# LuoGroup2023/PanTax

Hardware: AMD Instinct MI355X
Metric: PAO wall-time (s) + Mreads/s: packed reads + DB (graphs and their unique-trio index) resident in HBM -> abundance tables; the metric's own GAF -> abundance quantity is value_gaf_to_tables (files -> tables, never `value`) (higher is better)
Workload: dtype int64+f64

## Files before the change

include/pantax_hip.h:

```cpp
#ifndef PANTAX_HIP_H
#define PANTAX_HIP_H
#include <stddef.h>
#include <stdint.h>
#ifdef __cplusplus
extern "C" {
#endif

typedef enum {
    PANTAX_HIP_OK = 0,
    PANTAX_HIP_E_INVALID = -1,
    PANTAX_HIP_E_HIP = -2,
    PANTAX_HIP_E_NO_DEVICE = -3,
    PANTAX_HIP_E_LIMIT = -4,
    PANTAX_HIP_E_SOLVER = -5,
    PANTAX_HIP_E_IO = -6,
    PANTAX_HIP_E_STATE = -7
} pantax_hip_status;

typedef struct pantax_hip_ctx pantax_hip_ctx;
typedef struct pantax_hip_db pantax_hip_db;
typedef struct pantax_hip_reads pantax_hip_reads;

int pantax_hip_init(pantax_hip_ctx **out, const int *device_ids, int n_devices);
void pantax_hip_destroy(pantax_hip_ctx *ctx);
// ... 216 lines not shown
int pantax_hip_reads_load_gaf(pantax_hip_ctx *ctx, const char *path, pantax_hip_reads **reads_out, pantax_hip_gaf **gaf_out);
int pantax_hip_reads_set_flags(pantax_hip_ctx *ctx, pantax_hip_reads *reads, const uint8_t *flags);
void pantax_hip_gaf_free(pantax_hip_gaf *gaf);

typedef struct pantax_hip_graph pantax_hip_graph;
int pantax_hip_graph_load(const char *path, int format, pantax_hip_graph **out, const char **err_out);
int pantax_hip_graph_view(const pantax_hip_graph *g, uint64_t *n_nodes, uint64_t *n_haps, const int64_t **node_len,
                          const uint64_t **path_off, const uint32_t **path_nodes, const char *const **hap_names);
void pantax_hip_graph_free(pantax_hip_graph *g);

int pantax_hip_format_f64(double v, char *buf, size_t cap);

int pantax_hip_strain_node_stats(pantax_hip_ctx *ctx, pantax_hip_db *db, double *amax_out, uint32_t *nvalid_out, double *nzsum_out,
                                 uint32_t *nzcnt_out);

int pantax_hip_timing_enable(pantax_hip_ctx *ctx, int on);
int pantax_hip_timing_reset(pantax_hip_ctx *ctx);
int pantax_hip_timing_filter(pantax_hip_ctx *ctx, const char *name);
int pantax_hip_timing_get(pantax_hip_ctx *ctx, int cap, const char **names_out, uint64_t *launches_out,
                          double *total_ms_out);
int pantax_hip_sync(pantax_hip_ctx *ctx);

#ifdef __cplusplus
}
#endif
#endif
```

pantax_amd/_ffi.py:

```python
import ctypes as C
import os

import numpy as np

_HERE = os.path.dirname(os.path.abspath(__file__))
LIB_PATH = os.path.join(_HERE, "lib", "libpantax_hip.so")
_lib = None

SYMBOLS = [
    "pantax_hip_init", "pantax_hip_destroy", "pantax_hip_last_error", "pantax_hip_version", "pantax_hip_set_option",
    "pantax_hip_db_upload", "pantax_hip_db_upload_parts", "pantax_hip_db_free", "pantax_hip_reads_upload", "pantax_hip_reads_free",
    "pantax_hip_bin_reads", "pantax_hip_species_profile", "pantax_hip_db_reset", "pantax_hip_abundance_filter",
    "pantax_hip_trio_index", "pantax_hip_trio_get", "pantax_hip_node_coverage",
    "pantax_hip_strain_profile", "pantax_hip_strain_node_stats", "pantax_hip_pao_solve", "pantax_hip_pao_solve_batch", "pantax_hip_profile", "pantax_hip_profile_step", "pantax_hip_profile_step_enqueue", "pantax_hip_profile_step_collect", "pantax_hip_trio_index_prefetch", "pantax_hip_sort_rows",
    "pantax_hip_sample_ranks", "pantax_hip_chacha_block", "pantax_hip_gaf_filter", "pantax_hip_db_save_images", "pantax_hip_db_load_images",
    "pantax_hip_gaf_load", "pantax_hip_gaf_load_device", "pantax_hip_reads_load_gaf", "pantax_hip_reads_set_flags", "pantax_hip_gaf_view", "pantax_hip_gaf_free",
    "pantax_hip_graph_load", "pantax_hip_graph_view", "pantax_hip_graph_free", "pantax_hip_format_f64",
    "pantax_hip_read_strains", "pantax_hip_reads_route_pack", "pantax_hip_route_buffer", "pantax_hip_route_free", "pantax_hip_reads_from_routed",
    "pantax_hip_timing_enable", "pantax_hip_timing_filter", "pantax_hip_timing_reset", "pantax_hip_timing_get", "pantax_hip_sync",
]


class PantaxHipError(RuntimeError):
    def __init__(self, code, msg):
        super().__init__("pantax_hip error %d: %s" % (code, msg))
        self.code = code


class Graphs(C.Structure):
# ... 102 lines not shown
```

pantax_amd/csrc/api_core.cpp:

```cpp
#include <algorithm>
#include <chrono>
#include <cstdio>
#include <cstdlib>
#include <cstring>
#include <memory>
#include <numeric>
#include <string>
#include "common.hpp"

using namespace ptx;

extern "C" {

int pantax_hip_db_upload(pantax_hip_ctx *ctx, const pantax_hip_graphs *g, pantax_hip_db **out) {
    if (!ctx || !g || !out) return PANTAX_HIP_E_INVALID;
    *out = nullptr;
    PTX_ENTER(ctx);
    uint32_t S = g->n_species;
    if (S == 0) return fail(ctx, PANTAX_HIP_E_INVALID, "db_upload: n_species == 0");
    std::unique_ptr<pantax_hip_db> db(new pantax_hip_db());
    db->S = S;
    if (!g->node_len) {
        std::vector<uint32_t> order(S), rs(S), re(S);
        std::iota(order.begin(), order.end(), 0u);
// ... 290 lines not shown
    lap("node-block runs");
    PTX_TRY(node_haps_build(ctx, db));
    lap("node -> haplotypes");
    PTX_HIP(ctx, db->d_trio_first.alloc(1));
    PTX_HIP(ctx, db->d_trio_ent.alloc(2));
    PTX_HIP(ctx, db->d_trio_bases.alloc(1));
    PTX_HIP(ctx, db->d_active.alloc(S));
    PTX_HIP(ctx, hipStreamSynchronize(ctx->stream));
    return 0;
}

}

extern "C" {

void pantax_hip_db_free(pantax_hip_ctx *ctx, pantax_hip_db *db) {
    std::unique_lock<std::recursive_mutex> lk;
    if (ctx) lk = std::unique_lock<std::recursive_mutex>(ctx->mu);
    bool idle = false;
    if (ctx) {
        (void)hipSetDevice(ctx->device);
        idle = hipStreamSynchronize(ctx->stream) == hipSuccess;
        if (ctx->stream2) idle = hipStreamSynchronize(ctx->stream2) == hipSuccess && idle;
    }
    if (idle) { DevCacheIdleFrees scope; delete db; }
    else delete db;
}

int pantax_hip_reads_upload(pantax_hip_ctx *ctx, const pantax_hip_packed_reads *r, pantax_hip_reads **out) {
    if (!ctx || !r || !out) return PANTAX_HIP_E_INVALID;
// ... 92 lines not shown
```

pantax_amd/csrc/api_strain.cpp:

```cpp
#include <algorithm>
#include <chrono>
#include <cstdio>
#include <cstdlib>
#include <cmath>
#include <cstring>
#include <memory>
#include "lad.hpp"
#include "primitives.hpp"

using namespace ptx;

namespace {

inline double round2(double x) { return std::round(x * 100.0) / 100.0; }

struct StrainRaw {
    const uint32_t *nnz, *nvalid, *nzcnt, *sp_pat_off, *counts;
    const double *meanf, *amax, *nzsum, *x1, *x2, *obj1, *obj2;
    const int32_t *hap_bit, *sp_p, *st1, *st2, *it1, *it2;
    const uint8_t *fixed2, *need2;
    const unsigned long long *ratio;
};

struct ArenaLayout {
// ... 271 lines not shown

int pantax_hip_strain_node_stats(pantax_hip_ctx *ctx, pantax_hip_db *db, double *amax_out, uint32_t *nvalid_out, double *nzsum_out, uint32_t *nzcnt_out) {
    if (!ctx || !db) return PANTAX_HIP_E_INVALID;
    PTX_ENTER(ctx);
    if (db->stats_slot < 0 || db->h_arena[db->stats_slot].p == nullptr) return fail(ctx, PANTAX_HIP_E_STATE, "strain_node_stats: no strain step of this db has been collected");
    if (db->step_inflight) return fail(ctx, PANTAX_HIP_E_STATE, "strain_node_stats: %d enqueued step(s) of this db have not been collected (their download may reuse the slot)", db->step_inflight);
    const ArenaLayout L(db->S, db->H);
    const uint8_t *b = db->h_arena[db->stats_slot].p;
    if (amax_out) std::memcpy(amax_out, b + L.amax, sizeof(double) * db->S);
    if (nvalid_out) std::memcpy(nvalid_out, b + L.nvalid, sizeof(uint32_t) * db->S);
    if (nzsum_out) std::memcpy(nzsum_out, b + L.nzsum, sizeof(double) * db->S);
    if (nzcnt_out) std::memcpy(nzcnt_out, b + L.nzcnt, sizeof(uint32_t) * db->S);
    return 0;
}

int pantax_hip_pao_solve_batch(pantax_hip_ctx *ctx, const pantax_hip_species_batch *in, const pantax_hip_solution_batch *out) {
    if (!ctx || !in || !out || !in->node_off || !in->node_len || !in->node_abundance || !in->hap_off || !in->path_off || !in->path_nodes ||
        !in->cand_off || !in->cand_path_idx || !out->x || !out->status)
        return PANTAX_HIP_E_INVALID;
    const uint32_t S = in->n_species;
    if (S == 0) return fail(ctx, PANTAX_HIP_E_INVALID, "pao_solve_batch: n_species == 0");
    PTX_ENTER(ctx);
    const uint64_t V = in->node_off[S], H = in->hap_off[S];
    std::vector<int64_t> rs(S), re(S);
    for (uint32_t s = 0; s < S; ++s) {
        if (in->node_off[s + 1] <= in->node_off[s]) return fail(ctx, PANTAX_HIP_E_INVALID, "pao_solve_batch: species %u has no nodes", s);
        rs[s] = (int64_t)in->node_off[s] + 1; re[s] = (int64_t)in->node_off[s + 1];
    }
    pantax_hip_graphs g{S, rs.data(), re.data(), in->node_off, in->node_len, in->hap_off, in->path_off, in->path_nodes};
    pantax_hip_db *db = nullptr;
// ... 121 lines not shown
```

pantax_amd/csrc/common.hpp:

```cpp
#pragma once
#include <hip/hip_runtime.h>
#include <cstdint>
#include <cstdio>
#include <map>
#include <functional>
#include <mutex>
#include <cstring>
#include <atomic>
#include <string>
#include <vector>
#include "../../include/pantax_hip.h"

#ifndef TRIO_LH_PACK
#define TRIO_LH_PACK 0
#endif
namespace ptx {

struct Ctx;
#if TRIO_LH_PACK
using trio_len_t = uint2;
#else
using trio_len_t = uint32_t;
#endif

// ... 263 lines not shown
    DevBuf<uint32_t> d_node_base;
    DevBuf<uint64_t> d_bit_off;
    DevBuf<uint32_t> d_node_len;
    DevBuf<uint4> d_node_rec;
    DevBuf<uint64_t> d_path_off;
    DevBuf<uint32_t> d_path_nodes;
    DevBuf<uint32_t> d_hap_species;
    DevBuf<uint64_t> d_hap_off;
    DevBuf<uint8_t> d_all_same;
    std::vector<uint8_t> h_all_same;
    DevBuf<uint2> d_tiles;
    uint64_t n_tiles = 0;
    DevBuf<uint2> d_emit_tile_sp;
    DevBuf<uint64_t> d_node_haps;
    bool nh_built = false, nh_walk_too = false;
    DevBuf<uint32_t> d_tile_rank;
    DevBuf<uint32_t> d_hap_tile_off;
    bool trio_visit_ok = false;
    uint32_t n_vgroups = 0;
    std::vector<uint8_t> h_trio_slow;
    DevBuf<uint32_t> d_trio_slow;
    DevBuf<uint32_t> d_vis_pos;
    DevBuf<uint64_t> d_vis_head;
    DevBuf<uint32_t> d_vis_nbase;
    DevBuf<uint32_t> d_vis_sp;
    DevBuf<uint32_t> d_node_visited;
    bool trio_block_ok = false;
    uint32_t n_blocks = 0;
    uint64_t n_runs = 0;
    DevBuf<uint32_t> d_blk_base;
// ... 258 lines not shown
```

pantax_amd/csrc/primitives.hpp:

```cpp
#pragma once
#include "common.hpp"

namespace ptx {

size_t scan_tmp_elems(uint64_t n);
int exclusive_scan_u32(Ctx *ctx, const uint32_t *d_in, uint32_t *d_out, uint64_t n, uint32_t *d_tmp, uint32_t *d_total);
int exclusive_scan_u8(Ctx *ctx, const uint8_t *d_in, uint32_t *d_out, uint64_t n, uint32_t *d_tmp, uint32_t *d_total);

int zero_fill(Ctx *ctx, void *ptr, size_t bytes);
int byte_fill(Ctx *ctx, void *ptr, int byte, size_t bytes);

constexpr int SORT_MAX_WORDS = 3;
struct SortBufs {
    int nw = 0;
    uint64_t *k[SORT_MAX_WORDS] = {};
    uint32_t *v = nullptr;
};
struct SortPass {
    int word;
    int shift;
};
size_t sort_table_elems(uint64_t n);
int radix_sort(Ctx *ctx, SortBufs a, SortBufs b, uint64_t n, const SortPass *passes, int n_passes, uint32_t *d_table,
               uint32_t *d_scan_tmp, bool *result_in_b, const uint32_t *d_n = nullptr);
// ... 4 lines not shown
size_t sample_sort_ws_elems(uint64_t n_bound);
int sample_sort3(Ctx *ctx, SortBufs a, SortBufs b, uint64_t n_bound, uint32_t *d_ws, const uint32_t *d_n);

struct RowPatterns {
    uint64_t *pat_mask;
    uint32_t *pat_start, *pat_species, *sp_pat_off, *d_K;
    double *c0;
};
constexpr uint64_t SSN_MAX_SEG = 1ull << 26;
struct RowMaskSource {
    const unsigned long long *node_haps = nullptr;
    const uint64_t *hap_off = nullptr;
    const int32_t *hap_bit = nullptr, *sp_p = nullptr;
    const uint32_t *cov = nullptr, *node_len = nullptr;
    unsigned long long *ratio = nullptr;
    uint32_t max_haps = 0;
};
struct NodePartial { double mx, zs; unsigned long long nv, zc; };
struct NodeCovSource {
    const unsigned long long *bases = nullptr;
    const uint64_t *bit_off = nullptr;
    const uint32_t *full = nullptr, *bitmap = nullptr;
    const uint8_t *active = nullptr;
    double min_depth = 0.0;
    double *amax = nullptr, *nzsum = nullptr;
    uint32_t *nvalid = nullptr, *nzcnt = nullptr;
};
size_t sample_sort_nodes_ws_elems(uint32_t S, uint64_t seg_bound, uint64_t V);
int sample_sort_nodes(Ctx *ctx, const double *ab, const uint64_t *mask, const uint32_t *d_node_base, uint32_t S, uint64_t seg_bound, uint64_t V,
                      uint64_t *rows16, uint64_t *ksp, uint64_t *km, uint64_t *ka, int pack_shift, uint32_t *d_ws, uint32_t *d_n, const RowPatterns *pat = nullptr,
// ... 13 lines not shown
```

pantax_amd/csrc/sample_sort_nodes.hip:

```cpp
#include <algorithm>
#include <cstdio>
#include <cstdlib>
#include <vector>
#include "primitives.hpp"
#include "wave.hpp"

namespace ptx {

namespace {
#ifndef SN_LEVELS
#define SN_LEVELS 10
#endif
constexpr int SN_SAMPLE = 4096;
constexpr int SN_NLEAF = 1 << SN_LEVELS;
constexpr int SN_NSPLIT = SN_NLEAF - 1;
constexpr int SN_NBUCKET = 2 * SN_NLEAF;
#ifndef SN_ITEMS_N
#define SN_ITEMS_N 8
#endif
constexpr int SN_ITEMS = SN_ITEMS_N;
constexpr int SN_TILE = 256 * SN_ITEMS;
constexpr int SN_CAP = 4096;
constexpr int SN_WAVE_CAP = 512;
constexpr int SN_WAVE_CAP2 = 1024;
// ... 230 lines not shown
    uint32_t c = 0;
    for (uint32_t i = threadIdx.x; i < (uint32_t)SN_SAMPLE; i += 1024) c += ka[i] != ~0ull ? 1u : 0u;
    if (c) atomicAdd(&s_nv, c);
    __syncthreads();
    const uint32_t nv = s_nv;
    if (small) {
        for (uint32_t i = threadIdx.x; i < nv; i += 1024) sn.rows[o + i] = make_ulonglong2(km[i], ka[i]);
        if (threadIdx.x == 0) { sn.seg_n[s] = nv; w[SN_OFF_FLAGS + 3] = nv; }
        if (!sn.mask && sn.hp.ratio) {
            __shared__ unsigned long long s_r[128];
            if (threadIdx.x < 128) s_r[threadIdx.x] = 0;
            __syncthreads();
            for (uint32_t i = threadIdx.x; i < n; i += 1024) {
                uint64_t m = sn_node_mask(sn, s, o + i);
                const unsigned long long c = FUSED ? (m ? sn_node_cov<true>(sn, o + i) : 0u) : sn_node_cov<false>(sn, o + i), l = sn.hp.node_len[o + i];
                while (m) { const int k = __ffsll((long long)m) - 1; m &= m - 1; if (c) atomicAdd(&s_r[2 * k], c); atomicAdd(&s_r[2 * k + 1], l); }
            }
            __syncthreads();
            if (threadIdx.x < 128 && s_r[threadIdx.x]) atomicAdd(&sn.hp.ratio[2 * sn.hp.hap_off[s] + threadIdx.x], s_r[threadIdx.x]);
        }
        if (sn.c0) {
            __shared__ double s_c[16];
            double c = 0.0;
            for (uint32_t i = threadIdx.x; i < n; i += 1024) { const double av = sn_node_ab<FUSED>(sn, o + i); if (av > 0.0 && sn_node_mask(sn, s, o + i) == 0ull) c += av; }
            c = wave_reduce(c, [](double x, double y) { return x + y; });
            if ((threadIdx.x & 63) == 0) s_c[threadIdx.x >> 6] = c;
            __syncthreads();
            if (threadIdx.x == 0) { double t = 0.0; for (int q = 0; q < 16; ++q) t += s_c[q]; sn.c0[s] = t; }
        }
        return;
    }
// ... 150 lines not shown
#pragma unroll
        for (int k = 0; k < 8; ++k) {
            if (k >= p0) break;
            const unsigned long long cs = wave_reduce(c8[k], [](unsigned long long x, unsigned long long y) { return x + y; });
            const unsigned long long ls = wave_reduce(l8[k], [](unsigned long long x, unsigned long long y) { return x + y; });
            if (lane == 0) {
                if (cs) atomicAdd(&s_acc[2 * k], cs);
                if (ls) atomicAdd(&s_acc[2 * k + 1], ls);
            }
        }
        __syncthreads();
        if ((int)threadIdx.x < 2 * p0 && s_acc[threadIdx.x]) atomicAdd(&sn.hp.ratio[2 * h0 + threadIdx.x], s_acc[threadIdx.x]);
    }
}

constexpr int SN_HALF = SN_ITEMS >= 8 ? SN_ITEMS / 2 : SN_ITEMS;
static_assert(SN_ITEMS % SN_HALF == 0, "whole halves");
__global__ void __launch_bounds__(256) node_rows_kernel(Sn sn) {
    __shared__ ulonglong2 tree[SN_NLEAF];
    __shared__ uint32_t s_hist[SN_NBUCKET];
    extern __shared__ unsigned long long s_dyn_tab[];
    __shared__ int s_bit[64];
    __shared__ unsigned long long s_acc[2 * 64];
    const uint32_t s = blockIdx.y, g = blockIdx.x, o = sn.node_base[s], n = sn.node_base[s + 1] - o;
    uint32_t *w = sn.w(s);
    if (n == 0 || w[SN_OFF_FLAGS] != 0) return;
    uint32_t t0, t1;
    sn_tiles(sn, n, g, t0, t1);
    if (sn.skip_empty && sn.hp.sp_p[s] <= 0) {
        uint32_t *row0 = sn.cntm + ((size_t)s * sn.G + g) * SN_NBUCKET;
        for (int i = threadIdx.x; i < SN_NBUCKET; i += 256) row0[i] = 0u;
        if (threadIdx.x == 0) { sn.stage_cnt[(size_t)s * sn.G + g] = 0u; if (sn.c0) sn.c0p[(size_t)s * sn.G + g] = 0.0; }
        if (!sn.fz.active || sn.fz.active[s]) {
// ... 15 lines not shown
    if (t0 < t1) for (int i = threadIdx.x; i < SN_NLEAF; i += 256) tree[i] = gt[i];
    const uint64_t h0 = sn.hp.hap_off[s], nh = sn.hp.hap_off[s + 1] - h0;
    int p0 = sn.hp.sp_p[s];
    if (p0 <= 0 || p0 > 64 || nh > 64) p0 = 0;
    const int nbyte = p0 ? (int)((nh + 7) / 8) : 0;
    if (threadIdx.x < 64) s_bit[threadIdx.x] = (p0 && threadIdx.x < nh) ? sn.hp.hap_bit[h0 + threadIdx.x] : -1;
    if (threadIdx.x < 128) s_acc[threadIdx.x] = 0;
    __syncthreads();
    for (int b = 0; b < nbyte; ++b) {
        unsigned long long e = 0ull;
#pragma unroll
        for (int i = 0; i < 8; ++i) { const int bit = s_bit[8 * b + i]; if (((threadIdx.x >> i) & 1u) && bit >= 0) e |= 1ull << bit; }
        s_dyn_tab[b * 256 + threadIdx.x] = e;
    }
    __syncthreads();
    unsigned long long c8[8] = {0, 0, 0, 0, 0, 0, 0, 0}, l8[8] = {0, 0, 0, 0, 0, 0, 0, 0};
    const uint32_t stage0 = o + t0 * SN_TILE;
    const int lane = threadIdx.x & 63;
    const uint32_t wave64 = (uint32_t)__builtin_amdgcn_readfirstlane((int)(threadIdx.x >> 6)) << 6;
    double cacc = 0.0;
    NodeAcc nacc;
    constexpr int HALF = SN_HALF;
    for (uint32_t t = t0; t < t1; ++t) {
#pragma unroll
      for (int hb = 0; hb < SN_ITEMS; hb += HALF) {
        const uint32_t base = t * SN_TILE + (uint32_t)hb * 256u + threadIdx.x;
        double av[HALF];
        uint64_t mv[HALF];
        uint32_t cv[HALF], lv[HALF];
        {
            unsigned long long bs[HALF];
// ... 41 lines not shown
                    c = w0 == w1 ? __popc(bw0[r] & m0 & m1) : __popc(bw0[r] & m0) + __popc(bw1[r] & m1);
                    for (uint64_t ww = w0 + 1; ww < w1; ++ww) c += __popc(sn.fz.bitmap[ww]);
                }
                cv[r] = c;
                av[r] = 0.0;
                if (i < n) {
                    av[r] = (double)(long long)bs[r] / (double)lv[r];
                    nacc.add(av[r], sn.fz.min_depth);
                }
            }
        }
#pragma unroll
        for (int r = 0; r < HALF; ++r) {
            {
                const unsigned long long m = mv[r];
                if (m) {
                    const unsigned long long c = cv[r], l = lv[r];
#pragma unroll
                    for (int k = 0; k < 8; ++k)
                        if (k < p0) { const bool on = (m >> k) & 1ull; c8[k] += on ? c : 0ull; l8[k] += on ? l : 0ull; }
                    unsigned long long rest = m >> 8;
                    while (rest) {
                        const int k = __ffsll((long long)rest) - 1 + 8;
                        rest &= rest - 1;
                        if (c) atomicAdd(&s_acc[2 * k], c);
                        atomicAdd(&s_acc[2 * k + 1], l);
                    }
                }
            }
            uint32_t id = SN_NO_ROW;
            const uint64_t abits = (uint64_t)__double_as_longlong(av[r]);
            if (av[r] > 0.0 && mv[r] == 0ull) cacc += av[r];
            if (av[r] > 0.0 && mv[r] != 0ull) {
                const Key2 key{mv[r], abits};
                uint32_t k = 1;
#pragma unroll
                for (int l = 0; l < SN_LEVELS; ++l) { const ulonglong2 nd = tree[k]; k = 2u * k + (less2(Key2{nd.x, nd.y}, key) ? 1u : 0u); }
                const uint32_t lo = k - (uint32_t)SN_NLEAF;
                uint32_t eq = 0;
                if (lo < (uint32_t)SN_NSPLIT) { const ulonglong2 nd = tree[tree_node(lo)]; eq = eq2(Key2{nd.x, nd.y}, key) ? 1u : 0u; }
                id = 2u * lo + eq;
// ... 18 lines not shown
    sn_block_partial<4>(nacc, sn.npart + (size_t)s * sn.G + g);
    uint32_t *row = sn.cntm + ((size_t)s * sn.G + g) * SN_NBUCKET;
    for (int i = threadIdx.x; i < SN_NBUCKET; i += 256) row[i] = s_hist[i];
    if (threadIdx.x == 0) sn.stage_cnt[(size_t)s * sn.G + g] = s_nstage;
    if (sn.c0) {
        __shared__ double s_c[4];
        cacc = wave_reduce(cacc, [](double x, double y) { return x + y; });
        if (lane == 0) s_c[threadIdx.x >> 6] = cacc;
        __syncthreads();
        if (threadIdx.x == 0) sn.c0p[(size_t)s * sn.G + g] = (s_c[0] + s_c[1]) + (s_c[2] + s_c[3]);
    }
    if (p0 > 0 && sn.hp.ratio) {
#pragma unroll
        for (int k = 0; k < 8; ++k) {
            if (k >= p0) break;
            const unsigned long long cs = wave_reduce(c8[k], [](unsigned long long x, unsigned long long y) { return x + y; });
            const unsigned long long ls = wave_reduce(l8[k], [](unsigned long long x, unsigned long long y) { return x + y; });
            if (lane == 0) {
                if (cs) atomicAdd(&s_acc[2 * k], cs);
                if (ls) atomicAdd(&s_acc[2 * k + 1], ls);
            }
        }
        __syncthreads();
        if ((int)threadIdx.x < 2 * p0 && s_acc[threadIdx.x]) atomicAdd(&sn.hp.ratio[2 * h0 + threadIdx.x], s_acc[threadIdx.x]);
    }
}

__global__ void __launch_bounds__(64) node_rows_final_kernel(Sn sn) {
    const uint32_t s = blockIdx.x, n = sn.node_base[s + 1] - sn.node_base[s];
    double mx = -INFINITY, zs = 0.0; unsigned long long nv = 0, zc = 0;
    if (n != 0 && sn.fz.active && !sn.fz.active[s]) mx = 0.0;
    else if (n != 0) {
        const uint32_t nt = (n + SN_TILE - 1) / SN_TILE, ng = n <= (uint32_t)SN_SAMPLE ? 1u : (nt + sn.per - 1) / sn.per;
        for (uint32_t g = threadIdx.x; g < ng; g += 64) { const NodePartial p = sn.npart[(size_t)s * sn.G + g]; mx = fmax(mx, p.mx); zs += p.zs; nv += p.nv; zc += p.zc; }
    }
    mx = wave_reduce(mx, [](double x, double y) { return fmax(x, y); });
    zs = wave_reduce(zs, [](double x, double y) { return x + y; });
    nv = wave_reduce(nv, [](unsigned long long x, unsigned long long y) { return x + y; });
    zc = wave_reduce(zc, [](unsigned long long x, unsigned long long y) { return x + y; });
    if (threadIdx.x == 0) { sn.fz.amax[s] = mx; sn.fz.nvalid[s] = (uint32_t)nv; sn.fz.nzsum[s] = zs; sn.fz.nzcnt[s] = (uint32_t)zc; }
}

__global__ void __launch_bounds__(256) ssn_offsets_kernel(Sn sn) {
    __shared__ uint32_t s_wave[4];
    const uint32_t s = blockIdx.x, n = sn.node_base[s + 1] - sn.node_base[s];
    uint32_t *w = sn.w(s);
    if (n == 0 || w[SN_OFF_FLAGS] != 0) return;
    uint32_t *cm = sn.cntm + (size_t)s * sn.G * SN_NBUCKET;
    const uint32_t nt = (n + SN_TILE - 1) / SN_TILE, ng = (nt + sn.per - 1) / sn.per;
    constexpr int BPT = SN_NBUCKET / 256;
    static_assert(BPT % 4 == 0 && BPT >= 4, "16-byte steps");
    const uint32_t b0 = threadIdx.x * BPT;
    uint32_t tot[BPT], sum = 0;
#pragma unroll
    for (int i = 0; i < BPT; ++i) tot[i] = 0;
// ... 318 lines not shown
int sample_sort_nodes(Ctx *ctx, const double *ab, const uint64_t *mask, const uint32_t *d_node_base, uint32_t S, uint64_t seg_bound, uint64_t V,
                      uint64_t *rows16, uint64_t *ksp, uint64_t *km, uint64_t *ka, int pack_shift, uint32_t *d_ws, uint32_t *d_n, const RowPatterns *pat,
                      const RowMaskSource *haps, const NodeCovSource *fused) {
    if (S == 0 || V == 0) {
        PTX_HIP(ctx, hipMemsetAsync(d_n, 0, sizeof(uint32_t), ctx->stream));
        if (pat) { PTX_HIP(ctx, hipMemsetAsync(pat->d_K, 0, sizeof(uint32_t), ctx->stream)); PTX_HIP(ctx, hipMemsetAsync(pat->sp_pat_off, 0, (S + 1) * sizeof(uint32_t), ctx->stream));
                   PTX_HIP(ctx, hipMemsetAsync(pat->pat_start, 0, sizeof(uint32_t), ctx->stream)); }
        return 0;
    }
    if (seg_bound > SSN_MAX_SEG) return fail(ctx, PANTAX_HIP_E_LIMIT, "sample_sort_nodes: a segment of %llu nodes exceeds %llu", (unsigned long long)seg_bound, (unsigned long long)SSN_MAX_SEG);
    if (S > 65535) return fail(ctx, PANTAX_HIP_E_LIMIT, "sample_sort_nodes: %u segments exceed the launch grid", S);
    Sn sn;
    sn.node_base = d_node_base; sn.ab = ab; sn.mask = haps ? nullptr : mask; sn.ws = d_ws;
    if (haps) { if (haps->max_haps > 64) return fail(ctx, PANTAX_HIP_E_INVALID, "sample_sort_nodes: masks from haplotype words take species of at most 64 haplotypes"); sn.hp = *haps; }
    else if (!mask) return fail(ctx, PANTAX_HIP_E_INVALID, "sample_sort_nodes: neither a mask array nor haplotype words");
    if (fused && (!haps || !fused->bases || !fused->bit_off || !fused->full || !fused->bitmap || !fused->amax || !fused->nvalid || !fused->nzsum || !fused->nzcnt))
        return fail(ctx, PANTAX_HIP_E_INVALID, "sample_sort_nodes: the fused node pass takes haplotype words and the coverage arena");
    if (!fused && !ab) return fail(ctx, PANTAX_HIP_E_INVALID, "sample_sort_nodes: no abundance array");
    if (fused) { sn.fz = *fused; sn.ab = nullptr; sn.hp.cov = nullptr; }
    sn_geometry(S, seg_bound, &sn.G, &sn.per);
    sn.ablate = ctx->cfg.ssn_ablate;
    sn.skip_empty = ctx->cfg.no_absent_skip ? 0u : 1u;
    sn.cntm = d_ws + (size_t)S * SN_WS_WORDS;
    sn.stage_cnt = sn.cntm + (size_t)S * sn.G * SN_NBUCKET;
    uint32_t *cw = sn.stage_cnt + (size_t)S * sn.G;
    cw += ((reinterpret_cast<uintptr_t>(cw) & 7u) ? 1 : 0);
    sn.c0p = reinterpret_cast<double *>(cw);
    sn.c0 = pat ? pat->c0 : nullptr;
    uint32_t *tail = cw + 2 * (size_t)S * sn.G;
    sn.seg_n = tail; sn.seg_out = tail + S;
    uint32_t *sub_k = tail + 2 * (size_t)S + 4;
    sn.ids = reinterpret_cast<uint16_t *>(sub_k + (size_t)SN_NWH * S);
// ... 69 lines not shown
```

pantax_amd/csrc/stage_lad.hip:

```cpp
#include <algorithm>
#include <cstdio>
#include <vector>
#include "lad.hpp"
#include "row_sample.hpp"
#include "primitives.hpp"
#include "wave.hpp"
#include "scan_chained.hpp"

namespace ptx {

template <int NT>
__device__ __forceinline__ double block_sum_f64(double v, double *red) {
    v = wave_reduce(v, [](double x, double y) { return x + y; });
    const int lane = threadIdx.x & 63, wave = threadIdx.x >> 6;
    if (lane == 0) red[wave] = v;
    __syncthreads();
    double t = 0.0;
#pragma unroll
    for (int w = 0; w < NT / 64; ++w) t += red[w];
    __syncthreads();
    return t;
}
template <int NT>
__device__ __forceinline__ unsigned long long block_sum_u64(unsigned long long v, unsigned long long *red) {
// ... 1075 lines not shown
}
__global__ void __launch_bounds__(256) node_haps_ends_kernel(uint32_t H, const uint64_t *__restrict__ path_off, const uint32_t *__restrict__ path_nodes,
                                                             const uint32_t *__restrict__ hap_species, const uint32_t *__restrict__ node_base,
                                                             const uint64_t *__restrict__ hap_off, const uint32_t *__restrict__ slow,
                                                             unsigned long long *__restrict__ node_haps) {
    const uint32_t h = blockIdx.x * 256 + threadIdx.x;
    if (h >= H) return;
    const uint32_t sp = hap_species[h];
    if (slow[sp]) return;
    const uint64_t b = path_off[h], e = path_off[h + 1];
    if (e == b) return;
    const unsigned long long m = 1ull << (h - hap_off[sp]);
    atomicOr(&node_haps[node_base[sp] + path_nodes[b]], m);
    atomicOr(&node_haps[node_base[sp] + path_nodes[e - 1]], m);
}
bool use_node_haps(const Ctx *ctx, const Db *db) { return db->nh_built && ctx->cfg.mask != "walk"; }
int node_haps_build(Ctx *ctx, Db *db) {
    db->nh_built = false; db->nh_walk_too = false;
    const uint64_t V = db->V;
    if (!V || !db->P || !db->n_tiles) return 0;
    bool any_small = false;
    for (uint32_t s = 0; s < db->S; ++s) {
        if (db->h_hap_off[s + 1] - db->h_hap_off[s] > 64) db->nh_walk_too = true; else any_small = true;
    }
    if (!any_small) return 0;
    PTX_HIP(ctx, db->d_node_haps.alloc(V));
    PTX_TRY(zero_fill(ctx, db->d_node_haps.p, V * sizeof(uint64_t)));
    constexpr uint64_t NH_VISIT_HAPS = 16;
    const bool table = db->trio_visit_ok && db->n_vgroups && db->P < 0xFFFFFFFFull;
    std::vector<uint32_t> by_walk(db->S ? db->S : 1, 1u);
    bool any_walk = false, any_visits = false;
    for (uint32_t s = 0; s < db->S; ++s) {
        const uint64_t hs = db->h_hap_off[s + 1] - db->h_hap_off[s];
// ... 1 lines not shown
        if (hs <= 64) { if (by_walk[s]) any_walk = true; else any_visits = true; }
    }
    DevBuf<uint32_t> d_by_walk;
    PTX_TRY(upload(ctx, d_by_walk, by_walk.data(), by_walk.size()));
    if (any_visits) {
        hipLaunchKernelGGL(node_haps_visits_kernel, dim3((db->n_vgroups + 3) / 4), dim3(256), 0, ctx->stream, db->n_vgroups, db->d_vis_pos.p, db->d_vis_head.p, db->d_vis_nbase.p,
                           db->d_vis_sp.p, db->d_path_off.p, db->d_hap_off.p, db->d_path_nodes.p, (const uint32_t *)d_by_walk.p, (unsigned long long *)db->d_node_haps.p);
        hipLaunchKernelGGL(node_haps_ends_kernel, dim3((uint32_t)((db->H + 255) / 256)), dim3(256), 0, ctx->stream, (uint32_t)db->H, db->d_path_off.p, db->d_path_nodes.p,
                           db->d_hap_species.p, db->d_node_base.p, db->d_hap_off.p, (const uint32_t *)d_by_walk.p, (unsigned long long *)db->d_node_haps.p);
    }
    if (any_walk)
        hipLaunchKernelGGL(node_haps_fill_kernel, dim3((uint32_t)db->n_tiles), dim3(256), 0, ctx->stream, db->d_tiles.p, db->d_path_off.p, db->d_path_nodes.p,
                           db->d_hap_species.p, db->d_node_base.p, db->d_hap_off.p, (unsigned long long *)db->d_node_haps.p, 1u, (const uint32_t *)d_by_walk.p);
    PTX_HIP(ctx, hipStreamSynchronize(ctx->stream));
    PTX_HIP(ctx, hipGetLastError());
    db->nh_built = true;
    return 0;
}

static bool masks_in_sort_possible(const Ctx *ctx, const Db *db, bool *use_nodes_out, bool *ratio_by_node_out) {
    const uint32_t S = db->S;
    const uint64_t V = db->V;
    uint64_t max_vs = 0, max_hs = 0;
    for (uint32_t s_ = 0; s_ < S; ++s_) {
        max_vs = std::max<uint64_t>(max_vs, db->h_node_off[s_ + 1] - db->h_node_off[s_]);
        max_hs = std::max<uint64_t>(max_hs, db->h_hap_off[s_ + 1] - db->h_hap_off[s_]);
    }
    bool use_nodes = V > SS_MAX_N && max_vs <= SSN_MAX_SEG && S <= 65535;
    if (!ctx->cfg.row_sort.empty()) {
        const char *ev = ctx->cfg.row_sort.c_str();
        if (ev[0] == 'r') use_nodes = false;
        if (ev[0] == 'n') use_nodes = max_vs <= SSN_MAX_SEG && S <= 65535 && V > 0;
    }
    const bool ratio_by_node = use_node_haps(ctx, db) && V && !ctx->cfg.ratio_kernel;
    const bool wide = max_hs > (uint64_t)LAD_MAXP;
    const bool mask_pass_env = ctx->cfg.mask_pass || ctx->cfg.objective == "nodes";
    if (use_nodes_out) *use_nodes_out = use_nodes;
    if (ratio_by_node_out) *ratio_by_node_out = ratio_by_node;
    return use_nodes && ratio_by_node && !db->nh_walk_too && !wide && !mask_pass_env;
}

bool node_pass_fused_eligible(const Ctx *ctx, const Db *db, const pantax_hip_strain_config *cfg) {
    if (ctx->cfg.node_pass == "split" || !db->cov_count_pending || db->V == 0) return false;
    if (cfg->sample_nodes != 0 || ctx->cfg.cov_self_clean || db->cov_self_clean) return false;
    if (db->L / db->V >= (uint64_t)ctx->cfg.ncs_prefix_min && !ctx->cfg.ncs_no_prefix) return false;
    return masks_in_sort_possible(ctx, db, nullptr, nullptr);
}

int lad_prepare(Ctx *ctx, const Db *db, LadBatch *lb, bool cand_on_device, int pmax_bound) {
    const uint32_t S = db->S;
    lb->rows_c0_valid = false;
    const uint64_t V = db->V, H = db->H;
    if (!cand_on_device) {
        std::vector<int32_t> hap_bit(H ? H : 1, -1);
        for (uint32_t s = 0; s < S; ++s)
            for (int k = 0; k < lb->h_p[s]; ++k) hap_bit[db->h_hap_off[s] + lb->h_cand[db->h_hap_off[s] + k]] = k;
        PTX_TRY(upload(ctx, lb->d_hap_bit, hap_bit.data(), hap_bit.size()));
        PTX_TRY(upload(ctx, lb->d_p, lb->h_p.data(), S));
    }
    PTX_HIP(ctx, lb->d_mask.alloc(V));
// ... 107 lines not shown
        PTX_HIP(ctx, dbm->d_row16.alloc(4 * V));
        PTX_HIP(ctx, lb->d_c0.alloc(S));
        const RowPatterns pat{lb->d_pat_mask.p, lb->d_pat_start.p, lb->d_pat_species.p, lb->d_sp_pat_off.p, d_K, lb->d_c0.p};
        lb->rows_c0_valid = true;
        RowMaskSource hp;
        NodeCovSource fz;
        if (fused) {
            fz.bases = (const unsigned long long *)db->d_bases.p; fz.bit_off = db->d_bit_off.p; fz.full = db->d_full.p; fz.bitmap = db->d_bitmap.p;
            fz.active = lb->fused_active; fz.min_depth = lb->fused_min_depth;
            fz.amax = lb->d_amax.p; fz.nzsum = lb->d_nzsum.p; fz.nvalid = lb->d_nvalid.p; fz.nzcnt = lb->d_nzcnt.p;
        }
        if (masks_in_sort) {
            uint32_t mh = 0;
            for (uint32_t s_ = 0; s_ < S; ++s_) mh = std::max<uint32_t>(mh, (uint32_t)(db->h_hap_off[s_ + 1] - db->h_hap_off[s_]));
            hp.node_haps = (const unsigned long long *)db->d_node_haps.p; hp.hap_off = db->d_hap_off.p; hp.hap_bit = lb->d_hap_bit.p; hp.sp_p = lb->d_p.p;
            hp.cov = db->d_cov.p; hp.node_len = db->d_node_len.p; hp.ratio = lb->d_ratio.p; hp.max_haps = mh;
        }
        PTX_TRY(sample_sort_nodes(ctx, fused ? (const double *)nullptr : lb->d_ab.p, lb->d_mask.p, db->d_node_base.p, S, max_vs, V, dbm->d_row16.p, pack_shift >= 0 ? (uint64_t *)nullptr : ka[0].p,
                                  pack_shift >= 0 ? ka[0].p : ka[1].p, pack_shift >= 0 ? ka[1].p : ka[2].p, pack_shift, dbm->d_ss_ws.p, d_n, &pat, masks_in_sort ? &hp : nullptr,
                                  fused ? &fz : nullptr));
        if (fused) dbm->cov_count_pending = false;
    } else if (use_sample) {
        PTX_HIP(ctx, dbm->d_ss_ws.alloc(sample_sort_ws_elems(V)));
        PTX_TRY(sample_sort3(ctx, A, B, V, dbm->d_ss_ws.p, d_n));
    } else {
        std::vector<SortPass> passes;
        if (pack_shift >= 0) {
            add_passes(passes, 1, 0, 63);
            add_passes(passes, 0, 0, pmax_bound + sp_bits);
        } else {
            add_passes(passes, 2, 0, 63);
// ... 1254 lines not shown
```

pantax_amd/engine.py:

```python
import ctypes as C

import numpy as np

from . import _ffi
from ._ffi import PantaxHipError, as_c, p


class Engine:
    def __init__(self, device=0):
        self.lib = _ffi.load()
        self.ctx = C.c_void_p()
        dev = (C.c_int * 1)(device)
        rc = self.lib.pantax_hip_init(C.byref(self.ctx), dev, 1)
        if rc != 0:
            raise PantaxHipError(rc, self.lib.pantax_hip_last_error(None).decode())
        self.db = None
        self.reads = None
        self._keep = []
        self._step_buf = None
        self._collect_buf = None
        self._inflight = 0

    def _check(self, rc):
        if rc != 0:
# ... 472 lines not shown
        if _ffi.load().pantax_hip_chacha_block(p(key), C.c_uint64(counter), int(rounds), p(out)) != 0:
            raise ValueError("chacha_block")
        return out

    def sort_rows(self, k0, k1, k2, algo=0):
        k = [np.ascontiguousarray(x, dtype=np.uint64).copy() for x in (k0, k1, k2)]
        self._check(self.lib.pantax_hip_sort_rows(self.ctx, C.c_uint64(len(k[0])), p(k[0]), p(k[1]), p(k[2]), int(algo)))
        return k

    def strain_node_stats(self):
        amax, nzsum = np.zeros(self.S), np.zeros(self.S)
        nvalid, nzcnt = np.zeros(self.S, dtype=np.uint32), np.zeros(self.S, dtype=np.uint32)
        self._check(self.lib.pantax_hip_strain_node_stats(self.ctx, self.db, p(amax), p(nvalid), p(nzsum), p(nzcnt)))
        return amax, nvalid, nzsum, nzcnt

    def timing_enable(self, on=True):
        self._check(self.lib.pantax_hip_timing_enable(self.ctx, int(on)))

    def timing_filter(self, name=None):
        self._check(self.lib.pantax_hip_timing_filter(self.ctx, name.encode() if name else None))

    def timing_reset(self):
        self._check(self.lib.pantax_hip_timing_reset(self.ctx))

    def timing_get(self):
        cap = 256
        names = (C.c_char_p * cap)()
        launches = (C.c_uint64 * cap)()
        ms = (C.c_double * cap)()
        n = self.lib.pantax_hip_timing_get(self.ctx, cap, names, launches, ms)
# ... 20 lines not shown
```

Before: 6041.

## Precompute per-haplotype node length sums once and drop them from fused node pass

Result: no change. 6122, median of 6 (+1.3%).

```diff
diff --git a/include/pantax_hip.h b/include/pantax_hip.h
--- a/include/pantax_hip.h
+++ b/include/pantax_hip.h
@@ -254,6 +254,10 @@
 int pantax_hip_strain_node_stats(pantax_hip_ctx *ctx, pantax_hip_db *db, double *amax_out, uint32_t *nvalid_out, double *nzsum_out,
                                  uint32_t *nzcnt_out);
 
+int pantax_hip_strain_ratio_sums(pantax_hip_ctx *ctx, pantax_hip_db *db, uint64_t *sums_out);
+
+int pantax_hip_db_hap_node_len(pantax_hip_ctx *ctx, pantax_hip_db *db, uint64_t *out);
+
 int pantax_hip_timing_enable(pantax_hip_ctx *ctx, int on);
 int pantax_hip_timing_reset(pantax_hip_ctx *ctx);
 int pantax_hip_timing_filter(pantax_hip_ctx *ctx, const char *name);
diff --git a/pantax_amd/_ffi.py b/pantax_amd/_ffi.py
--- a/pantax_amd/_ffi.py
+++ b/pantax_amd/_ffi.py
@@ -12,7 +12,7 @@
     "pantax_hip_db_upload", "pantax_hip_db_upload_parts", "pantax_hip_db_free", "pantax_hip_reads_upload", "pantax_hip_reads_free",
     "pantax_hip_bin_reads", "pantax_hip_species_profile", "pantax_hip_db_reset", "pantax_hip_abundance_filter",
     "pantax_hip_trio_index", "pantax_hip_trio_get", "pantax_hip_node_coverage",
-    "pantax_hip_strain_profile", "pantax_hip_strain_node_stats", "pantax_hip_pao_solve", "pantax_hip_pao_solve_batch", "pantax_hip_profile", "pantax_hip_profile_step", "pantax_hip_profile_step_enqueue", "pantax_hip_profile_step_collect", "pantax_hip_trio_index_prefetch", "pantax_hip_sort_rows",
+    "pantax_hip_strain_profile", "pantax_hip_strain_node_stats", "pantax_hip_strain_ratio_sums", "pantax_hip_db_hap_node_len", "pantax_hip_pao_solve", "pantax_hip_pao_solve_batch", "pantax_hip_profile", "pantax_hip_profile_step", "pantax_hip_profile_step_enqueue", "pantax_hip_profile_step_collect", "pantax_hip_trio_index_prefetch", "pantax_hip_sort_rows",
     "pantax_hip_sample_ranks", "pantax_hip_chacha_block", "pantax_hip_gaf_filter", "pantax_hip_db_save_images", "pantax_hip_db_load_images",
     "pantax_hip_gaf_load", "pantax_hip_gaf_load_device", "pantax_hip_reads_load_gaf", "pantax_hip_reads_set_flags", "pantax_hip_gaf_view", "pantax_hip_gaf_free",
     "pantax_hip_graph_load", "pantax_hip_graph_view", "pantax_hip_graph_free", "pantax_hip_format_f64",
diff --git a/pantax_amd/csrc/api_core.cpp b/pantax_amd/csrc/api_core.cpp
--- a/pantax_amd/csrc/api_core.cpp
+++ b/pantax_amd/csrc/api_core.cpp
@@ -328,6 +328,14 @@
 
 extern "C" {
 
+int pantax_hip_db_hap_node_len(pantax_hip_ctx *ctx, pantax_hip_db *db, uint64_t *out) {
+    if (!ctx || !db || !out) return PANTAX_HIP_E_INVALID;
+    PTX_ENTER(ctx);
+    if (db->h_hap_len.size() != db->H) return fail(ctx, PANTAX_HIP_E_STATE, "db_hap_node_len: the table of this db was not built");
+    if (db->H) std::memcpy(out, db->h_hap_len.data(), sizeof(uint64_t) * db->H);
+    return 0;
+}
+
 void pantax_hip_db_free(pantax_hip_ctx *ctx, pantax_hip_db *db) {
     std::unique_lock<std::recursive_mutex> lk;
     if (ctx) lk = std::unique_lock<std::recursive_mutex>(ctx->mu);
diff --git a/pantax_amd/csrc/api_strain.cpp b/pantax_amd/csrc/api_strain.cpp
--- a/pantax_amd/csrc/api_strain.cpp
+++ b/pantax_amd/csrc/api_strain.cpp
@@ -309,6 +309,16 @@
     return 0;
 }
 
+int pantax_hip_strain_ratio_sums(pantax_hip_ctx *ctx, pantax_hip_db *db, uint64_t *sums_out) {
+    if (!ctx || !db || !sums_out) return PANTAX_HIP_E_INVALID;
+    PTX_ENTER(ctx);
+    if (db->stats_slot < 0 || db->h_arena[db->stats_slot].p == nullptr) return fail(ctx, PANTAX_HIP_E_STATE, "strain_ratio_sums: no strain step of this db has been collected");
+    if (db->step_inflight) return fail(ctx, PANTAX_HIP_E_STATE, "strain_ratio_sums: %d enqueued step(s) of this db have not been collected (their download may reuse the slot)", db->step_inflight);
+    const ArenaLayout L(db->S, db->H);
+    std::memcpy(sums_out, db->h_arena[db->stats_slot].p + L.ratio, sizeof(uint64_t) * 2 * db->H);
+    return 0;
+}
+
 int pantax_hip_pao_solve_batch(pantax_hip_ctx *ctx, const pantax_hip_species_batch *in, const pantax_hip_solution_batch *out) {
     if (!ctx || !in || !out || !in->node_off || !in->node_len || !in->node_abundance || !in->hap_off || !in->path_off || !in->path_nodes ||
         !in->cand_off || !in->cand_path_idx || !out->x || !out->status)
diff --git a/pantax_amd/csrc/common.hpp b/pantax_amd/csrc/common.hpp
--- a/pantax_amd/csrc/common.hpp
+++ b/pantax_amd/csrc/common.hpp
@@ -301,6 +301,9 @@
     DevBuf<uint2> d_emit_tile_sp;
     DevBuf<uint64_t> d_node_haps;
     bool nh_built = false, nh_walk_too = false;
+    DevBuf<uint64_t> d_hap_len;
+    std::vector<uint64_t> h_hap_len;
+    uint64_t max_species_bases = 0;
     DevBuf<uint32_t> d_tile_rank;
     DevBuf<uint32_t> d_hap_tile_off;
     bool trio_visit_ok = false;
diff --git a/pantax_amd/csrc/primitives.hpp b/pantax_amd/csrc/primitives.hpp
--- a/pantax_amd/csrc/primitives.hpp
+++ b/pantax_amd/csrc/primitives.hpp
@@ -42,6 +42,7 @@
     const int32_t *hap_bit = nullptr, *sp_p = nullptr;
     const uint32_t *cov = nullptr, *node_len = nullptr;
     unsigned long long *ratio = nullptr;
+    const uint64_t *hap_len = nullptr;
     uint32_t max_haps = 0;
 };
 struct NodePartial { double mx, zs; unsigned long long nv, zc; };
diff --git a/pantax_amd/csrc/sample_sort_nodes.hip b/pantax_amd/csrc/sample_sort_nodes.hip
--- a/pantax_amd/csrc/sample_sort_nodes.hip
+++ b/pantax_amd/csrc/sample_sort_nodes.hip
@@ -268,7 +268,11 @@
             for (uint32_t i = threadIdx.x; i < n; i += 1024) {
                 uint64_t m = sn_node_mask(sn, s, o + i);
                 const unsigned long long c = FUSED ? (m ? sn_node_cov<true>(sn, o + i) : 0u) : sn_node_cov<false>(sn, o + i), l = sn.hp.node_len[o + i];
-                while (m) { const int k = __ffsll((long long)m) - 1; m &= m - 1; if (c) atomicAdd(&s_r[2 * k], c); atomicAdd(&s_r[2 * k + 1], l); }
+                while (m) {
+                    const int k = __ffsll((long long)m) - 1; m &= m - 1;
+                    if (c) atomicAdd(&s_r[2 * k], c);
+                    if constexpr (!FUSED) atomicAdd(&s_r[2 * k + 1], l);
+                }
             }
             __syncthreads();
             if (threadIdx.x < 128 && s_r[threadIdx.x]) atomicAdd(&sn.hp.ratio[2 * sn.hp.hap_off[s] + threadIdx.x], s_r[threadIdx.x]);
@@ -449,9 +453,15 @@
     }
 }
 
-constexpr int SN_HALF = SN_ITEMS >= 8 ? SN_ITEMS / 2 : SN_ITEMS;
+#ifndef SN_ROWS_HALF
+#define SN_ROWS_HALF (SN_ITEMS >= 8 ? SN_ITEMS / 2 : SN_ITEMS)
+#endif
+#ifndef SN_ROWS_WAVES
+#define SN_ROWS_WAVES 5
+#endif
+constexpr int SN_HALF = SN_ROWS_HALF;
 static_assert(SN_ITEMS % SN_HALF == 0, "whole halves");
-__global__ void __launch_bounds__(256) node_rows_kernel(Sn sn) {
+__global__ void __launch_bounds__(256, SN_ROWS_WAVES) node_rows_kernel(Sn sn) {
     __shared__ ulonglong2 tree[SN_NLEAF];
     __shared__ uint32_t s_hist[SN_NBUCKET];
     extern __shared__ unsigned long long s_dyn_tab[];
@@ -497,7 +507,7 @@
         s_dyn_tab[b * 256 + threadIdx.x] = e;
     }
     __syncthreads();
-    unsigned long long c8[8] = {0, 0, 0, 0, 0, 0, 0, 0}, l8[8] = {0, 0, 0, 0, 0, 0, 0, 0};
+    uint32_t c8[8] = {0, 0, 0, 0, 0, 0, 0, 0};
     const uint32_t stage0 = o + t0 * SN_TILE;
     const int lane = threadIdx.x & 63;
     const uint32_t wave64 = (uint32_t)__builtin_amdgcn_readfirstlane((int)(threadIdx.x >> 6)) << 6;
@@ -569,17 +579,16 @@
         for (int r = 0; r < HALF; ++r) {
             {
                 const unsigned long long m = mv[r];
-                if (m) {
-                    const unsigned long long c = cv[r], l = lv[r];
+                const uint32_t c = cv[r];
+                if (m && c) {
 #pragma unroll
                     for (int k = 0; k < 8; ++k)
-                        if (k < p0) { const bool on = (m >> k) & 1ull; c8[k] += on ? c : 0ull; l8[k] += on ? l : 0ull; }
+                        if (k < p0) c8[k] += ((m >> k) & 1ull) ? c : 0u;
                     unsigned long long rest = m >> 8;
                     while (rest) {
                         const int k = __ffsll((long long)rest) - 1 + 8;
                         rest &= rest - 1;
-                        if (c) atomicAdd(&s_acc[2 * k], c);
-                        atomicAdd(&s_acc[2 * k + 1], l);
+                        atomicAdd(&s_acc[2 * k], (unsigned long long)c);
                     }
                 }
             }
@@ -628,15 +637,11 @@
 #pragma unroll
         for (int k = 0; k < 8; ++k) {
             if (k >= p0) break;
-            const unsigned long long cs = wave_reduce(c8[k], [](unsigned long long x, unsigned long long y) { return x + y; });
-            const unsigned long long ls = wave_reduce(l8[k], [](unsigned long long x, unsigned long long y) { return x + y; });
-            if (lane == 0) {
-                if (cs) atomicAdd(&s_acc[2 * k], cs);
-                if (ls) atomicAdd(&s_acc[2 * k + 1], ls);
-            }
+            const unsigned long long cs = wave_reduce((unsigned long long)c8[k], [](unsigned long long x, unsigned long long y) { return x + y; });
+            if (lane == 0 && cs) atomicAdd(&s_acc[2 * k], cs);
         }
         __syncthreads();
-        if ((int)threadIdx.x < 2 * p0 && s_acc[threadIdx.x]) atomicAdd(&sn.hp.ratio[2 * h0 + threadIdx.x], s_acc[threadIdx.x]);
+        if ((int)threadIdx.x < p0 && s_acc[2 * threadIdx.x]) atomicAdd(&sn.hp.ratio[2 * (h0 + threadIdx.x)], s_acc[2 * threadIdx.x]);
     }
 }
 
@@ -653,6 +658,14 @@
     nv = wave_reduce(nv, [](unsigned long long x, unsigned long long y) { return x + y; });
     zc = wave_reduce(zc, [](unsigned long long x, unsigned long long y) { return x + y; });
     if (threadIdx.x == 0) { sn.fz.amax[s] = mx; sn.fz.nvalid[s] = (uint32_t)nv; sn.fz.nzsum[s] = zs; sn.fz.nzcnt[s] = (uint32_t)zc; }
+    if (sn.hp.ratio) {
+        const uint64_t h0 = sn.hp.hap_off[s], nh = sn.hp.hap_off[s + 1] - h0;
+        const int p = sn.hp.sp_p[s];
+        if (p > 0 && p <= 64 && nh <= 64 && threadIdx.x < nh) {
+            const int k = sn.hp.hap_bit[h0 + threadIdx.x];
+            if (k >= 0 && k < p) sn.hp.ratio[2 * (h0 + (uint64_t)k) + 1] = sn.hp.hap_len[h0 + threadIdx.x];
+        }
+    }
 }
 
 __global__ void __launch_bounds__(256) ssn_offsets_kernel(Sn sn) {
@@ -1001,8 +1014,8 @@
     sn.node_base = d_node_base; sn.ab = ab; sn.mask = haps ? nullptr : mask; sn.ws = d_ws;
     if (haps) { if (haps->max_haps > 64) return fail(ctx, PANTAX_HIP_E_INVALID, "sample_sort_nodes: masks from haplotype words take species of at most 64 haplotypes"); sn.hp = *haps; }
     else if (!mask) return fail(ctx, PANTAX_HIP_E_INVALID, "sample_sort_nodes: neither a mask array nor haplotype words");
-    if (fused && (!haps || !fused->bases || !fused->bit_off || !fused->full || !fused->bitmap || !fused->amax || !fused->nvalid || !fused->nzsum || !fused->nzcnt))
-        return fail(ctx, PANTAX_HIP_E_INVALID, "sample_sort_nodes: the fused node pass takes haplotype words and the coverage arena");
+    if (fused && (!haps || !haps->hap_len || !fused->bases || !fused->bit_off || !fused->full || !fused->bitmap || !fused->amax || !fused->nvalid || !fused->nzsum || !fused->nzcnt))
+        return fail(ctx, PANTAX_HIP_E_INVALID, "sample_sort_nodes: the fused node pass takes haplotype words, the haplotype length table and the coverage arena");
     if (!fused && !ab) return fail(ctx, PANTAX_HIP_E_INVALID, "sample_sort_nodes: no abundance array");
     if (fused) { sn.fz = *fused; sn.ab = nullptr; sn.hp.cov = nullptr; }
     sn_geometry(S, seg_bound, &sn.G, &sn.per);
diff --git a/pantax_amd/csrc/stage_lad.hip b/pantax_amd/csrc/stage_lad.hip
--- a/pantax_amd/csrc/stage_lad.hip
+++ b/pantax_amd/csrc/stage_lad.hip
@@ -1113,9 +1113,70 @@
     atomicOr(&node_haps[node_base[sp] + path_nodes[b]], m);
     atomicOr(&node_haps[node_base[sp] + path_nodes[e - 1]], m);
 }
+__global__ void __launch_bounds__(256) hap_len_kernel(uint64_t V, const uint2 *__restrict__ tile_sp, const uint32_t *__restrict__ node_base,
+                                                      const uint64_t *__restrict__ hap_off, const unsigned long long *__restrict__ node_haps,
+                                                      const uint32_t *__restrict__ node_len, unsigned long long *__restrict__ hap_len) {
+    __shared__ unsigned long long acc[64];
+    const uint64_t v0 = (uint64_t)blockIdx.x * 2048;
+    const uint2 t = tile_sp[blockIdx.x];
+    const uint32_t sp0 = t.x;
+    const uint64_t h0 = hap_off[sp0], nh_all = hap_off[sp0 + 1] - h0;
+    const int nh = nh_all <= 64 ? (int)nh_all : 0;
+    const uint64_t end0 = sp0 < t.y ? (uint64_t)node_base[sp0 + 1] : V;
+    if (threadIdx.x < 64) acc[threadIdx.x] = 0;
+    __syncthreads();
+    unsigned long long hm[8];
+    uint32_t l[8];
+#pragma unroll
+    for (int r = 0; r < 8; ++r) {
+        const uint64_t v = v0 + (uint64_t)r * 256 + threadIdx.x;
+        hm[r] = 0; l[r] = 0;
+        if (v < V) { hm[r] = node_haps[v]; l[r] = node_len[v]; }
+        if (v < V && v >= end0) {
+            uint32_t sp = sp0 + 1;
+            while (sp < t.y && node_base[sp + 1] <= v) ++sp;
+            unsigned long long m = hm[r];
+            while (m) { const int j = __ffsll((long long)m) - 1; m &= m - 1; atomicAdd(&hap_len[hap_off[sp] + j], (unsigned long long)l[r]); }
+            hm[r] = 0;
+        }
+    }
+    for (int j = 0; j < nh; ++j) {
+        unsigned long long x = 0;
+#pragma unroll
+        for (int r = 0; r < 8; ++r) x += ((hm[r] >> j) & 1ull) ? l[r] : 0u;
+        x = wave_reduce(x, [](unsigned long long a, unsigned long long b) { return a + b; });
+        if ((threadIdx.x & 63) == 0 && x) atomicAdd(&acc[j], x);
+    }
+    __syncthreads();
+    if ((int)threadIdx.x < nh && acc[threadIdx.x]) atomicAdd(&hap_len[h0 + threadIdx.x], acc[threadIdx.x]);
+}
+__global__ void __launch_bounds__(256) species_bit0_kernel(uint32_t S, const uint32_t *__restrict__ node_base, const uint64_t *__restrict__ bit_off, uint64_t *__restrict__ out) {
+    const uint32_t s = blockIdx.x * 256 + threadIdx.x;
+    if (s <= S) out[s] = bit_off[node_base[s]];
+}
+static int hap_len_build(Ctx *ctx, Db *db) {
+    const uint64_t V = db->V, H = db->H;
+    const uint32_t S = db->S;
+    PTX_HIP(ctx, db->d_hap_len.alloc(H ? H : 1));
+    PTX_TRY(zero_fill(ctx, db->d_hap_len.p, (H ? H : 1) * sizeof(uint64_t)));
+    hipLaunchKernelGGL(hap_len_kernel, dim3((uint32_t)((V + 2047) / 2048)), dim3(256), 0, ctx->stream, V, db->d_emit_tile_sp.p, db->d_node_base.p, db->d_hap_off.p,
+                       (const unsigned long long *)db->d_node_haps.p, db->d_node_len.p, (unsigned long long *)db->d_hap_len.p);
+    DevBuf<uint64_t> d_b0;
+    PTX_HIP(ctx, d_b0.alloc((size_t)S + 1));
+    hipLaunchKernelGGL(species_bit0_kernel, dim3((S + 1 + 255) / 256), dim3(256), 0, ctx->stream, S, db->d_node_base.p, db->d_bit_off.p, d_b0.p);
+    PTX_HIP(ctx, hipGetLastError());
+    std::vector<uint64_t> b0((size_t)S + 1);
+    PTX_TRY(download(ctx, db->h_hap_len.data(), db->d_hap_len.p, H));
+    PTX_TRY(download(ctx, b0.data(), d_b0.p, (size_t)S + 1));
+    PTX_HIP(ctx, hipStreamSynchronize(ctx->stream));
+    db->max_species_bases = 0;
+    for (uint32_t s = 0; s < S; ++s) db->max_species_bases = std::max<uint64_t>(db->max_species_bases, b0[s + 1] - b0[s]);
+    return 0;
+}
 bool use_node_haps(const Ctx *ctx, const Db *db) { return db->nh_built && ctx->cfg.mask != "walk"; }
 int node_haps_build(Ctx *ctx, Db *db) {
     db->nh_built = false; db->nh_walk_too = false;
+    db->h_hap_len.assign(db->H, 0ull); db->max_species_bases = 0;
     const uint64_t V = db->V;
     if (!V || !db->P || !db->n_tiles) return 0;
     bool any_small = false;
@@ -1147,6 +1208,7 @@
                            db->d_hap_species.p, db->d_node_base.p, db->d_hap_off.p, (unsigned long long *)db->d_node_haps.p, 1u, (const uint32_t *)d_by_walk.p);
     PTX_HIP(ctx, hipStreamSynchronize(ctx->stream));
     PTX_HIP(ctx, hipGetLastError());
+    PTX_TRY(hap_len_build(ctx, db));
     db->nh_built = true;
     return 0;
 }
@@ -1177,6 +1239,7 @@
     if (ctx->cfg.node_pass == "split" || !db->cov_count_pending || db->V == 0) return false;
     if (cfg->sample_nodes != 0 || ctx->cfg.cov_self_clean || db->cov_self_clean) return false;
     if (db->L / db->V >= (uint64_t)ctx->cfg.ncs_prefix_min && !ctx->cfg.ncs_no_prefix) return false;
+    if (!db->d_hap_len.p || db->max_species_bases > 0xFFFFFFFFull) return false;
     return masks_in_sort_possible(ctx, db, nullptr, nullptr);
 }
 
@@ -1314,7 +1377,7 @@
             uint32_t mh = 0;
             for (uint32_t s_ = 0; s_ < S; ++s_) mh = std::max<uint32_t>(mh, (uint32_t)(db->h_hap_off[s_ + 1] - db->h_hap_off[s_]));
             hp.node_haps = (const unsigned long long *)db->d_node_haps.p; hp.hap_off = db->d_hap_off.p; hp.hap_bit = lb->d_hap_bit.p; hp.sp_p = lb->d_p.p;
-            hp.cov = db->d_cov.p; hp.node_len = db->d_node_len.p; hp.ratio = lb->d_ratio.p; hp.max_haps = mh;
+            hp.cov = db->d_cov.p; hp.node_len = db->d_node_len.p; hp.ratio = lb->d_ratio.p; hp.max_haps = mh; hp.hap_len = db->d_hap_len.p;
         }
         PTX_TRY(sample_sort_nodes(ctx, fused ? (const double *)nullptr : lb->d_ab.p, lb->d_mask.p, db->d_node_base.p, S, max_vs, V, dbm->d_row16.p, pack_shift >= 0 ? (uint64_t *)nullptr : ka[0].p,
                                   pack_shift >= 0 ? ka[0].p : ka[1].p, pack_shift >= 0 ? ka[1].p : ka[2].p, pack_shift, dbm->d_ss_ws.p, d_n, &pat, masks_in_sort ? &hp : nullptr,
diff --git a/pantax_amd/engine.py b/pantax_amd/engine.py
--- a/pantax_amd/engine.py
+++ b/pantax_amd/engine.py
@@ -510,6 +510,16 @@
         self._check(self.lib.pantax_hip_strain_node_stats(self.ctx, self.db, p(amax), p(nvalid), p(nzsum), p(nzcnt)))
         return amax, nvalid, nzsum, nzcnt
 
+    def strain_ratio_sums(self):
+        out = np.zeros((self.H, 2), dtype=np.uint64)
+        self._check(self.lib.pantax_hip_strain_ratio_sums(self.ctx, self.db, p(out)))
+        return out
+
+    def db_hap_node_len(self):
+        out = np.zeros(self.H, dtype=np.uint64)
+        self._check(self.lib.pantax_hip_db_hap_node_len(self.ctx, self.db, p(out)))
+        return out
+
     def timing_enable(self, on=True):
         self._check(self.lib.pantax_hip_timing_enable(self.ctx, int(on)))
 
```
